# TritonDataCenter/containerpilot

Measured on AMD Instinct MI355X. Metric: events/sec, higher is better.
Workload: dtype n/a (CPU daemon, no tensor math; see BASELINE.json north_star); 1 GPU; model=containerpilot daemon, BASELINE stress shape scaled to 550 jobs, jobs=550, watches=50, parallelism=1 independent daemons (1/rank)

## Files before the change

### cpp/include/cpilot/loop.hpp

```cpp
#pragma once

#include <sys/types.h>

#include <chrono>
#include <cstdint>
#include <deque>
#include <functional>
#include <map>
#include <memory>
#include <mutex>
#include <queue>
#include <vector>

namespace cpilot {

using Clock = std::chrono::steady_clock;
using TimePoint = Clock::time_point;
using Ns = std::chrono::nanoseconds;

std::function<void()> timedItem(const char* tag, std::function<void()> fn);
void dumpItemTags();

void resetThreadScheduling();

class Loop {
 public:
  using FdCallback = std::function<void(uint32_t epollEvents)>;
  using TimerCallback = std::function<void()>;
  using ChildCallback = std::function<void(int waitStatus)>;

  Loop();
  ~Loop();

  Loop(const Loop&) = delete;
  Loop& operator=(const Loop&) = delete;

  void watchFd(int fd, uint32_t events, FdCallback cb);
  void modifyFd(int fd, uint32_t events);
  void unwatchFd(int fd);

  uint64_t addTimeout(Ns delay, TimerCallback cb);
  uint64_t addInterval(Ns interval, TimerCallback cb, Ns initialDelay = Ns(-1));
  void cancelTimer(uint64_t id);

  void defer(std::function<void()> fn);

  void post(std::function<void()> fn);

  void watchChild(pid_t pid, ChildCallback cb);
  void reapChildren();
  void notifyChildExit(pid_t pid, int status);

  static void postIfLive(Loop* loop, uint64_t id, std::function<void()> fn);
  uint64_t id() const { return id_; }

  void run();
  void stop();

  bool stopped() const { return stopped_; }

 private:
  struct Timer {
    uint64_t id;
    TimePoint deadline;
    Ns interval;
    TimerCallback cb;
    bool canceled = false;
  };
  struct TimerCmp {
    bool operator()(const std::shared_ptr<Timer>& a,
                    const std::shared_ptr<Timer>& b) const {
      return a->deadline > b->deadline;
    }
  };

  void armTimerFd();
  void fireDueTimers();
  void drainDeferred();
  void drainPosted();

  uint64_t id_ = 0;
  int epfd_ = -1;
  int timerfd_ = -1;
  int wakeupFds_[2] = {-1, -1};
  bool stopped_ = false;

  std::map<int, FdCallback> fdCallbacks_;
  std::priority_queue<std::shared_ptr<Timer>,
                      std::vector<std::shared_ptr<Timer>>, TimerCmp>
      timers_;
  std::map<uint64_t, std::shared_ptr<Timer>> timersById_;
  uint64_t nextTimerId_ = 1;

  std::deque<std::function<void()>> deferred_;

  std::mutex postedMu_;
  std::deque<std::function<void()>> posted_;

  std::map<pid_t, ChildCallback> children_;
  std::map<pid_t, int> unclaimedExits_;
};

}
```

### cpp/src/command.cpp

```cpp
#include "cpilot/command.hpp"

#include <fcntl.h>
#include <signal.h>
#include <sys/epoll.h>
#include <sys/wait.h>
#include <unistd.h>

#include <cctype>
#include <cstring>
#include <cstdio>
#include <map>

#include "cpilot/log.hpp"
#include "cpilot/spawner.hpp"

extern char** environ;

namespace cpilot {

namespace {

std::map<std::string, std::string>& pidEnvOverlay() {
  static std::map<std::string, std::string> overlay;
  return overlay;
}

std::shared_ptr<const std::vector<std::string>>& baseEnvCache() {
  static std::shared_ptr<const std::vector<std::string>> cache;
  return cache;
}
bool& baseEnvDirty() {
  static bool dirty = true;
  return dirty;
}

std::shared_ptr<const std::vector<std::string>> baseEnvSnapshot() {
  if (!baseEnvDirty() && baseEnvCache()) return baseEnvCache();
  auto& overlay = pidEnvOverlay();
  auto env = std::make_shared<std::vector<std::string>>();
  for (char** e = ::environ; *e; e++) {
    const char* eq = strchr(*e, '=');
    if (eq && overlay.count(std::string(*e, eq - *e))) continue;
    env->emplace_back(*e);
  }
  baseEnvCache() = env;
  baseEnvDirty() = false;
  return baseEnvCache();
}

std::vector<std::string>& overlayStrings() {
  static std::vector<std::string> strings;
  return strings;
}
std::map<std::string, size_t>& overlayIndex() {
  static std::map<std::string, size_t> index;
  return index;
}

const std::vector<std::string>& overlayExtras() { return overlayStrings(); }

void overlaySet(const std::string& key, const std::string& value) {
  auto [it, inserted] = pidEnvOverlay().emplace(key, value);
  if (inserted) {
    overlayIndex()[key] = overlayStrings().size();
    overlayStrings().push_back(key + "=" + value);
    if (getenv(key.c_str())) baseEnvDirty() = true;
  } else {
    it->second = value;
    overlayStrings()[overlayIndex()[key]] = key + "=" + value;
  }
}

void overlayErase(const std::string& key) {
  if (pidEnvOverlay().erase(key)) {
    auto idxIt = overlayIndex().find(key);
    if (idxIt != overlayIndex().end()) {
      size_t slot = idxIt->second;
      overlayIndex().erase(idxIt);
      auto& strs = overlayStrings();
      if (slot + 1 != strs.size()) {
        strs[slot] = std::move(strs.back());
        size_t eq = strs[slot].find('=');
        overlayIndex()[strs[slot].substr(0, eq)] = slot;
      }
      strs.pop_back();
    }
    if (getenv(key.c_str())) baseEnvDirty() = true;
  }
}

}

void commandEnvInvalidate() { baseEnvDirty() = true; }

bool parseArgs(const Json& raw, std::string* execPath,
               std::vector<std::string>* args, std::string* err) {
  std::vector<std::string> all;
  if (raw.isString()) {
    std::string s = raw.str();
    size_t a = 0, b = s.size();
    while (a < b && isspace((unsigned char)s[a])) a++;
    while (b > a && isspace((unsigned char)s[b - 1])) b--;
    s = s.substr(a, b - a);
    if (!s.empty()) {
      std::string cur;
      for (char c : s) {
        if (c == ' ') {
          all.push_back(cur);
          cur.clear();
        } else {
          cur += c;
        }
      }
      all.push_back(cur);
    }
  } else if (raw.isArray()) {
    for (auto& e : raw.array()) {
      if (e.isString()) all.push_back(e.str());
      else all.push_back(e.dump());
    }
  } else if (!raw.isNull()) {
    *err = "unable to parse exec arguments";
    return false;
  }
  if (all.empty()) {
    *err = "received zero-length argument";
    return false;
  }
  *execPath = all[0];
  args->assign(all.begin() + 1, all.end());
  return true;
}

CommandPtr newCommand(const Json& rawExec, Duration timeout, bool raw,
                      const std::string& logField, std::string* err) {
  std::string execPath;
  std::vector<std::string> args;
  if (!parseArgs(rawExec, &execPath, &args, err)) return nullptr;
  return std::make_shared<Command>(execPath, args, timeout, raw, logField);
}

Command::Command(std::string execPath, std::vector<std::string> args,
                 Duration timeout, bool raw, std::string logField)
    : name_(execPath),
      exec_(std::move(execPath)),
      args_(std::move(args)),
      timeout_(timeout),
      raw_(raw),
      logField_(std::move(logField)) {}

std::string Command::envName() const {
  if (name_.empty()) return name_;
  std::string name = name_;
  size_t slash = name.find_last_of('/');
  if (slash != std::string::npos) name = name.substr(slash + 1);
  size_t dot = name.find_last_of('.');
  if (dot != std::string::npos && dot > 0)
    name = name.substr(0, dot) + name.substr(name.size());
  std::string out;
  for (char c : name) {
    if (isalnum((unsigned char)c)) {
      out += (char)toupper((unsigned char)c);
    } else if (out.empty() || out.back() != '_') {
      out += '_';
    }
  }
  return out;
}

void Command::run(Loop& loop, std::shared_ptr<Bus> bus) {
  if (running_) {
    LOG_DEBUG("%s already running, queueing run", name_.c_str());
    pendingRun_ = true;
    return;
  }
  spawn(loop, std::move(bus));
}

void Command::spawn(Loop& loop, std::shared_ptr<Bus> bus) {
  loop_ = &loop;
  LOG_DEBUG("%s.Run start", name_.c_str());

  int pipefds[2] = {-1, -1};
  if (!raw_) {
    if (pipe2(pipefds, O_CLOEXEC) != 0) {
      LOG_ERROR("unable to create pipe for %s: %s", name_.c_str(),
                strerror(errno));
      bus->publish(Event{EventCode::ExitFailed, name_});
      bus->publish(Event{EventCode::Error, strerror(errno)});
      return;
    }
  }

  running_ = true;
  pid_ = -1;
  pendingSignal_ = 0;
  tReq_ = Clock::now();
  auto self = shared_from_this();
  int readFd = pipefds[0];
  auto baseEnv = baseEnvSnapshot();
  Spawner::SpawnCb compCb =
      [this, self, bus, readFd](pid_t pid, int err) {
        if (pid < 0) {
          LOG_ERROR("unable to start %s: %s", name_.c_str(), strerror(err));
          if (readFd >= 0) close(readFd);
          running_ = false;
          pendingRun_ = false;
          pendingSignal_ = 0;
          bus->publish(Event{EventCode::ExitFailed, name_});
          bus->publish(Event{EventCode::Error, strerror(err)});
          return;
        }
        pid_ = pid;
        tCb_ = Clock::now();
        if (pidEnvName_.empty())
          pidEnvName_ = "CONTAINERPILOT_" + envName() + "_PID";
        overlaySet(pidEnvName_, std::to_string(pid));

        if (!raw_) {
          logFd_ = readFd;
          fcntl(logFd_, F_SETFL, O_NONBLOCK);
          loop_->watchFd(logFd_, EPOLLIN | EPOLLHUP, [this, self](uint32_t) {
            char buf[4096];
            while (true) {
              ssize_t n = read(logFd_, buf, sizeof(buf));
              if (n > 0) {
                logBuf_.append(buf, n);
                size_t pos;
                while ((pos = logBuf_.find('\n')) != std::string::npos) {
                  logging::logFields(logging::Level::Info, logField_, pid_,
                                     logBuf_.substr(0, pos));
                  logBuf_.erase(0, pos + 1);
                }
              } else if (n == 0 || (n < 0 && errno != EAGAIN)) {
                if (!logBuf_.empty()) {
                  logging::logFields(logging::Level::Info, logField_, pid_,
                                     logBuf_);
                  logBuf_.clear();
                }
                loop_->unwatchFd(logFd_);
                close(logFd_);
                logFd_ = -1;
                return;
              } else {
                return;
              }
            }
          });
        }

        if (timeout_ > Duration(0)) {
          timeoutTimer_ = loop_->addTimeout(timeout_, [this, self] {
            LOG_WARN("%s timeout after %llds", name_.c_str(),
                     (long long)std::chrono::duration_cast<
                         std::chrono::seconds>(timeout_)
                         .count());
            timeoutTimer_ = 0;
            kill();
          });
        }

        if (pendingSignal_ != 0) {
          ::kill(-pid, pendingSignal_);
          pendingSignal_ = 0;
        }

        loop_->watchChild(pid, [this, self, bus](int status) {
          onExit(*loop_, bus, status);
        });
      };
  Spawner::global().spawn(loop, exec_, args_, std::move(baseEnv),
                          overlayExtras(), raw_ ? -1 : pipefds[1],
                          std::move(compCb));
}

void Command::onExit(Loop& loop, std::shared_ptr<Bus> bus, int status) {
  LOG_DEBUG("%s.Run end", name_.c_str());
  static const bool rttDebug = cpilotDebugEnv("CPILOT_LOOP_DEBUG");
  if (rttDebug) {
    auto now = Clock::now();
    double total =
        std::chrono::duration<double, std::milli>(now - tReq_).count();
    if (total > 50.0) {
      double execPhase =
          std::chrono::duration<double, std::milli>(now - tCb_).count();
      fprintf(stderr,
              "spawn rtt: %s total=%.0fms spawn_phase=%.0fms "
              "exec_phase=%.0fms\n",
              name_.c_str(), total, total - execPhase, execPhase);
    }
  }
  if (timeoutTimer_) {
    loop.cancelTimer(timeoutTimer_);
    timeoutTimer_ = 0;
  }
  if (logFd_ >= 0) {
    char buf[4096];
    ssize_t n;
    while ((n = read(logFd_, buf, sizeof(buf))) > 0) logBuf_.append(buf, n);
    size_t pos;
    while ((pos = logBuf_.find('\n')) != std::string::npos) {
      logging::logFields(logging::Level::Info, logField_, pid_,
                         logBuf_.substr(0, pos));
      logBuf_.erase(0, pos + 1);
    }
    if (!logBuf_.empty()) {
      logging::logFields(logging::Level::Info, logField_, pid_, logBuf_);
      logBuf_.clear();
    }
    loop.unwatchFd(logFd_);
    close(logFd_);
    logFd_ = -1;
  }

  if (!pidEnvName_.empty()) overlayErase(pidEnvName_);

  running_ = false;
  pid_ = -1;

  bool success = WIFEXITED(status) && WEXITSTATUS(status) == 0;
  if (success) {
    LOG_DEBUG("%s exited without error", name_.c_str());
    bus->publish(Event{EventCode::ExitSuccess, name_});
  } else {
    int code = WIFEXITED(status) ? WEXITSTATUS(status)
                                 : 128 + (WIFSIGNALED(status) ? WTERMSIG(status) : 0);
    LOG_ERROR("%s exited with error: exit status %d", name_.c_str(), code);
    bus->publish(Event{EventCode::ExitFailed, name_});
    bus->publish(Event{EventCode::Error,
                      name_ + ": exit status " + std::to_string(code)});
  }

  if (pendingRun_) {
    pendingRun_ = false;
    spawn(loop, bus);
  }
}

void Command::term() {
  LOG_DEBUG("%s.term", name_.c_str());
  if (pid_ > 0) {
    LOG_DEBUG("terminating command '%s' at pid: %d", name_.c_str(), pid_);
    ::kill(-pid_, SIGTERM);
  } else if (running_ && pendingSignal_ != SIGKILL) {
    pendingSignal_ = SIGTERM;
  }
}

void Command::kill() {
  LOG_DEBUG("%s.kill", name_.c_str());
  if (pid_ > 0) {
    LOG_DEBUG("killing command '%s' at pid: %d", name_.c_str(), pid_);
    ::kill(-pid_, SIGKILL);
  } else if (running_) {
    pendingSignal_ = SIGKILL;
  }
}

}
```

### cpp/src/loop.cpp

```cpp
#include "cpilot/loop.hpp"

#include <fcntl.h>
#include <sched.h>
#include <sys/resource.h>
#include <sys/epoll.h>
#include <sys/timerfd.h>
#include <sys/wait.h>
#include <unistd.h>

#include <cstdio>
#include <cstring>
#include <algorithm>
#include <set>
#include <stdexcept>

#include "cpilot/log.hpp"

namespace cpilot {

void resetThreadScheduling() {
  struct sched_param sp;
  memset(&sp, 0, sizeof(sp));
  sched_setscheduler(0, SCHED_OTHER, &sp);
  setpriority(PRIO_PROCESS, 0, 0);
}

namespace {
std::mutex& liveLoopsMu() {
  static std::mutex mu;
  return mu;
}
std::map<Loop*, uint64_t>& liveLoops() {
  static std::map<Loop*, uint64_t> loops;
  return loops;
}
uint64_t nextLoopId() {
  static uint64_t next = 1;
  return next++;
}
}

namespace {
struct ItemTagStats {
  double ms = 0;
  uint64_t count = 0;
};
std::map<std::string, ItemTagStats>& itemTags() {
  static std::map<std::string, ItemTagStats> tags;
  return tags;
}
}

std::function<void()> timedItem(const char* tag, std::function<void()> fn) {
  static const bool on = cpilotDebugEnv("CPILOT_LOOP_DEBUG");
  if (!on) return fn;
  std::string t(tag);
  return [t, fn = std::move(fn)] {
    TimePoint t0 = Clock::now();
    fn();
    auto& slot = itemTags()[t];
    slot.ms +=
        std::chrono::duration<double, std::milli>(Clock::now() - t0).count();
    slot.count++;
  };
}

void dumpItemTags() {
  for (auto& kv : itemTags())
    fprintf(stderr, "  item tag %s: %.0fms over %llu (avg %.1fus)\n",
            kv.first.c_str(), kv.second.ms,
            (unsigned long long)kv.second.count,
            kv.second.count ? kv.second.ms * 1000 / kv.second.count : 0.0);
  itemTags().clear();
}

void Loop::postIfLive(Loop* loop, uint64_t id, std::function<void()> fn) {
  std::lock_guard<std::mutex> l(liveLoopsMu());
  auto it = liveLoops().find(loop);
  if (it != liveLoops().end() && it->second == id) loop->post(std::move(fn));
}

Loop::Loop() {
  {
    std::lock_guard<std::mutex> l(liveLoopsMu());
    id_ = nextLoopId();
    liveLoops()[this] = id_;
  }
  epfd_ = epoll_create1(EPOLL_CLOEXEC);
  if (epfd_ < 0) throw std::runtime_error("epoll_create1 failed");
  timerfd_ = timerfd_create(CLOCK_MONOTONIC, TFD_NONBLOCK | TFD_CLOEXEC);
  if (timerfd_ < 0) throw std::runtime_error("timerfd_create failed");
  if (pipe2(wakeupFds_, O_NONBLOCK | O_CLOEXEC) != 0)
    throw std::runtime_error("pipe2 failed");

  watchFd(timerfd_, EPOLLIN, [this](uint32_t) {
    uint64_t expirations;
    while (read(timerfd_, &expirations, sizeof(expirations)) > 0) {
    }
    fireDueTimers();
  });
  watchFd(wakeupFds_[0], EPOLLIN, [this](uint32_t) {
    char buf[256];
    while (read(wakeupFds_[0], buf, sizeof(buf)) > 0) {
    }
    drainPosted();
  });
}

Loop::~Loop() {
  {
    std::lock_guard<std::mutex> l(liveLoopsMu());
    liveLoops().erase(this);
  }
  if (epfd_ >= 0) close(epfd_);
  if (timerfd_ >= 0) close(timerfd_);
  if (wakeupFds_[0] >= 0) close(wakeupFds_[0]);
  if (wakeupFds_[1] >= 0) close(wakeupFds_[1]);
}

void Loop::watchFd(int fd, uint32_t events, FdCallback cb) {
  struct epoll_event ev;
  memset(&ev, 0, sizeof(ev));
  ev.events = events;
  ev.data.fd = fd;
  if (epoll_ctl(epfd_, EPOLL_CTL_ADD, fd, &ev) != 0)
    throw std::runtime_error(std::string("epoll_ctl ADD failed: ") +
                             strerror(errno));
  fdCallbacks_[fd] = std::move(cb);
}

void Loop::modifyFd(int fd, uint32_t events) {
  struct epoll_event ev;
  memset(&ev, 0, sizeof(ev));
  ev.events = events;
  ev.data.fd = fd;
  epoll_ctl(epfd_, EPOLL_CTL_MOD, fd, &ev);
}

void Loop::unwatchFd(int fd) {
  epoll_ctl(epfd_, EPOLL_CTL_DEL, fd, nullptr);
  fdCallbacks_.erase(fd);
}

uint64_t Loop::addTimeout(Ns delay, TimerCallback cb) {
  auto t = std::make_shared<Timer>();
  t->id = nextTimerId_++;
  t->deadline = Clock::now() + delay;
  t->interval = Ns(0);
  t->cb = std::move(cb);
  timersById_[t->id] = t;
  timers_.push(t);
  armTimerFd();
  return t->id;
}

uint64_t Loop::addInterval(Ns interval, TimerCallback cb, Ns initialDelay) {
  if (interval <= Ns(0)) interval = Ns(1);
  if (initialDelay < Ns(0)) initialDelay = interval;
  auto t = std::make_shared<Timer>();
  t->id = nextTimerId_++;
  t->deadline = Clock::now() + initialDelay;
  t->interval = interval;
  t->cb = std::move(cb);
  timersById_[t->id] = t;
  timers_.push(t);
  armTimerFd();
  return t->id;
}

void Loop::cancelTimer(uint64_t id) {
  auto it = timersById_.find(id);
  if (it == timersById_.end()) return;
  it->second->canceled = true;
  timersById_.erase(it);
}

void Loop::defer(std::function<void()> fn) { deferred_.push_back(std::move(fn)); }

void Loop::post(std::function<void()> fn) {
  {
    std::lock_guard<std::mutex> l(postedMu_);
    posted_.push_back(std::move(fn));
  }
  char b = 1;
  ssize_t unused = write(wakeupFds_[1], &b, 1);
  (void)unused;
}

void Loop::watchChild(pid_t pid, ChildCallback cb) {
  auto it = unclaimedExits_.find(pid);
  if (it != unclaimedExits_.end()) {
    int status = it->second;
    unclaimedExits_.erase(it);
    cb(status);
    return;
  }
  children_[pid] = std::move(cb);
}

void Loop::reapChildren() {
  constexpr int kReapBatch = 64;
  int n = 0;
  while (n < kReapBatch) {
    int status = 0;
    pid_t pid = waitpid(-1, &status, WNOHANG);
    if (pid <= 0) return;
    n++;
    notifyChildExit(pid, status);
  }
  defer([this] { reapChildren(); });
}

void Loop::notifyChildExit(pid_t pid, int status) {
  auto it = children_.find(pid);
  if (it != children_.end()) {
    ChildCallback cb = std::move(it->second);
    children_.erase(it);
    cb(status);
  } else {
    unclaimedExits_[pid] = status;
  }
}

void Loop::armTimerFd() {
  while (!timers_.empty() && timers_.top()->canceled) timers_.pop();
  struct itimerspec its;
  memset(&its, 0, sizeof(its));
  if (!timers_.empty()) {
    auto now = Clock::now();
    Ns delta = std::chrono::duration_cast<Ns>(timers_.top()->deadline - now);
    if (delta < Ns(1)) delta = Ns(1);
    its.it_value.tv_sec = delta.count() / 1000000000LL;
    its.it_value.tv_nsec = delta.count() % 1000000000LL;
  }
  timerfd_settime(timerfd_, 0, &its, nullptr);
}

void Loop::fireDueTimers() {
  static const bool stallDebug = cpilotDebugEnv("CPILOT_LOOP_DEBUG");
  auto timeCb = [](Timer* t, const TimerCallback& cb) {
    if (!stallDebug) { cb(); return; }
    TimePoint t0 = Clock::now();
    cb();
    auto ms = std::chrono::duration<double, std::milli>(Clock::now() - t0)
                  .count();
    if (ms > 10.0)
      fprintf(stderr, "timer stall: id=%llu interval_ms=%lld took %.1f ms\n",
              (unsigned long long)t->id,
              (long long)(t->interval.count() / 1000000), ms);
  };
  auto now = Clock::now();
  while (!timers_.empty()) {
    auto t = timers_.top();
    if (t->canceled) {
      timers_.pop();
      continue;
    }
    if (t->deadline > now) break;
    timers_.pop();
    if (t->interval > Ns(0)) {
      t->deadline += t->interval;
      if (t->deadline <= now) {
        auto behind = std::chrono::duration_cast<Ns>(now - t->deadline);
        auto periods = behind.count() / t->interval.count() + 1;
        t->deadline += Ns(periods * t->interval.count());
      }
      timers_.push(t);
      timeCb(t.get(), t->cb);
    } else {
      auto keep = t;
      timersById_.erase(t->id);
      timeCb(keep.get(), keep->cb);
    }
  }
  armTimerFd();
}

void Loop::drainDeferred() {
  size_t n = deferred_.size();
  for (size_t i = 0; i < n && !deferred_.empty(); i++) {
    auto fn = std::move(deferred_.front());
    deferred_.pop_front();
    fn();
  }
}

void Loop::drainPosted() {
  constexpr auto kBudget = std::chrono::milliseconds(2);
  constexpr size_t kHardCap = 4096;
  TimePoint start = Clock::now();
  size_t processed = 0;
  bool more = true;
  while (more && processed < kHardCap &&
         Clock::now() - start < kBudget) {
    std::deque<std::function<void()>> batch;
    {
      std::lock_guard<std::mutex> l(postedMu_);
      for (size_t i = 0; i < 64 && !posted_.empty(); i++) {
        batch.push_back(std::move(posted_.front()));
        posted_.pop_front();
      }
      more = !posted_.empty();
    }
    static const bool itemDebug = cpilotDebugEnv("CPILOT_LOOP_DEBUG");
    if (itemDebug) {
      static double accMs = 0;
      static uint64_t nItems = 0, nSlow = 0;
      static TimePoint lastDump = Clock::now();
      for (auto& fn : batch) {
        TimePoint ti = Clock::now();
        fn();
        double ms = std::chrono::duration<double, std::milli>(
                        Clock::now() - ti).count();
        accMs += ms;
        nItems++;
        if (ms > 0.2) nSlow++;
      }
      if (Clock::now() - lastDump > std::chrono::seconds(5)) {
        fprintf(stderr,
                "posted items: %llu in 5s, total=%.0fms avg=%.1fus "
                "slow(>200us)=%llu\n",
                (unsigned long long)nItems, accMs,
                nItems ? accMs * 1000.0 / nItems : 0.0,
                (unsigned long long)nSlow);
        accMs = 0;
        nItems = nSlow = 0;
        lastDump = Clock::now();
      }
    } else {
      for (auto& fn : batch) fn();
    }
    processed += batch.size();
    if (batch.empty()) break;
  }
  if (more) {
    char b = 1;
    ssize_t unused = write(wakeupFds_[1], &b, 1);
    (void)unused;
  }
}

void Loop::run() {
  stopped_ = false;
  const bool stallDebug = cpilotDebugEnv("CPILOT_LOOP_DEBUG");
  auto probe = [stallDebug](const char* phase, TimePoint t0, int fd = -1) {
    if (!stallDebug) return;
    auto ms = std::chrono::duration<double, std::milli>(Clock::now() - t0)
                  .count();
    if (ms > 10.0)
      fprintf(stderr, "loop stall: %s fd=%d took %.1f ms\n", phase, fd, ms);
  };
  std::vector<struct epoll_event> events(64);
  double accDeferred = 0, accEpoll = 0, accFds = 0, accTimers = 0;
  std::map<int, std::pair<double, uint64_t>> accPerFd;
  uint64_t iters = 0;
  TimePoint lastReport = Clock::now();
  auto acc = [](double* slot, TimePoint t0) {
    *slot += std::chrono::duration<double, std::milli>(Clock::now() - t0)
                 .count();
  };
  while (!stopped_) {
    TimePoint t0 = Clock::now();
    drainDeferred();
    probe("drainDeferred", t0);
    if (stallDebug) acc(&accDeferred, t0);
    if (stopped_) break;
    armTimerFd();
    int timeoutMs = deferred_.empty() ? 1000 : 0;
    TimePoint te = Clock::now();
    int n = epoll_wait(epfd_, events.data(), (int)events.size(), timeoutMs);
    if (stallDebug) acc(&accEpoll, te);
    if (n < 0) {
      if (errno == EINTR) continue;
      LOG_ERROR("epoll_wait: %s", strerror(errno));
      break;
    }
    TimePoint tf = Clock::now();
    for (int i = 0; i < n && !stopped_; i++) {
      int fd = events[i].data.fd;
      auto it = fdCallbacks_.find(fd);
      if (it != fdCallbacks_.end()) {
        FdCallback cb = it->second;
        TimePoint tc = Clock::now();
        cb(events[i].events);
        probe("fdCallback", tc, fd);
        if (stallDebug) {
          auto& slot = accPerFd[fd];
          slot.first += std::chrono::duration<double, std::milli>(
                            Clock::now() - tc).count();
          slot.second++;
        }
      }
    }
    if (stallDebug) acc(&accFds, tf);
    TimePoint tt = Clock::now();
    fireDueTimers();
    probe("fireDueTimers", tt);
    if (stallDebug) {
      acc(&accTimers, tt);
      iters++;
      if (Clock::now() - lastReport > std::chrono::seconds(5)) {
        double secs = std::chrono::duration<double>(Clock::now() -
                                                    lastReport).count();
        fprintf(stderr,
                "loop phases: %.0f it/s deferred=%.0fms epoll=%.0fms "
                "fds=%.0fms timers=%.0fms (per %.1fs)\n",
                iters / secs, accDeferred, accEpoll, accFds, accTimers,
                secs);
        std::vector<std::pair<double, std::pair<int, uint64_t>>> top;
        for (auto& kv : accPerFd)
          top.push_back({kv.second.first, {kv.first, kv.second.second}});
        std::sort(top.rbegin(), top.rend());
        for (size_t k = 0; k < top.size() && k < 4; k++)
          fprintf(stderr, "  top fd %d: %.0fms over %llu events\n",
                  top[k].second.first, top[k].first,
                  (unsigned long long)top[k].second.second);
        dumpItemTags();
        accPerFd.clear();
        accDeferred = accEpoll = accFds = accTimers = 0;
        iters = 0;
        lastReport = Clock::now();
      }
    }
  }
}

void Loop::stop() { stopped_ = true; }

}
```

Before: 11000 events/s.

## Skip redundant timerfd rearming and cheapen PID env overlay updates

```diff
diff --git a/cpp/include/cpilot/loop.hpp b/cpp/include/cpilot/loop.hpp
--- a/cpp/include/cpilot/loop.hpp
+++ b/cpp/include/cpilot/loop.hpp
@@ -59,6 +59,8 @@
 
   bool stopped() const { return stopped_; }
 
+  uint64_t timerArmCount() const { return timerArmCount_; }
+
  private:
   struct Timer {
     uint64_t id;
@@ -91,6 +93,8 @@
       timers_;
   std::map<uint64_t, std::shared_ptr<Timer>> timersById_;
   uint64_t nextTimerId_ = 1;
+  int64_t armedDeadlineNs_ = 0;
+  uint64_t timerArmCount_ = 0;
 
   std::deque<std::function<void()>> deferred_;
 
diff --git a/cpp/src/command.cpp b/cpp/src/command.cpp
--- a/cpp/src/command.cpp
+++ b/cpp/src/command.cpp
@@ -9,7 +9,7 @@
 #include <cctype>
 #include <cstring>
 #include <cstdio>
-#include <map>
+#include <unordered_map>
 
 #include "cpilot/log.hpp"
 #include "cpilot/spawner.hpp"
@@ -20,9 +20,31 @@
 
 namespace {
 
-std::map<std::string, std::string>& pidEnvOverlay() {
-  static std::map<std::string, std::string> overlay;
-  return overlay;
+struct OverlaySlot {
+  static constexpr size_t kAbsent = (size_t)-1;
+  size_t index = kAbsent;
+  std::string parked;
+  int inEnviron = -1;
+};
+std::unordered_map<std::string, OverlaySlot>& overlaySlots() {
+  static std::unordered_map<std::string, OverlaySlot> slots;
+  return slots;
+}
+std::vector<std::string>& overlayStrings() {
+  static std::vector<std::string> strings;
+  return strings;
+}
+std::vector<OverlaySlot*>& overlayOwners() {
+  static std::vector<OverlaySlot*> owners;
+  return owners;
+}
+
+const std::vector<std::string>& overlayExtras() { return overlayStrings(); }
+
+bool overlayHas(const std::string& key) {
+  auto it = overlaySlots().find(key);
+  return it != overlaySlots().end() &&
+         it->second.index != OverlaySlot::kAbsent;
 }
 
 std::shared_ptr<const std::vector<std::string>>& baseEnvCache() {
@@ -36,11 +58,10 @@
 
 std::shared_ptr<const std::vector<std::string>> baseEnvSnapshot() {
   if (!baseEnvDirty() && baseEnvCache()) return baseEnvCache();
-  auto& overlay = pidEnvOverlay();
   auto env = std::make_shared<std::vector<std::string>>();
   for (char** e = ::environ; *e; e++) {
     const char* eq = strchr(*e, '=');
-    if (eq && overlay.count(std::string(*e, eq - *e))) continue;
+    if (eq && overlayHas(std::string(*e, eq - *e))) continue;
     env->emplace_back(*e);
   }
   baseEnvCache() = env;
@@ -48,51 +69,65 @@
   return baseEnvCache();
 }
 
-std::vector<std::string>& overlayStrings() {
-  static std::vector<std::string> strings;
-  return strings;
-}
-std::map<std::string, size_t>& overlayIndex() {
-  static std::map<std::string, size_t> index;
-  return index;
-}
-
-const std::vector<std::string>& overlayExtras() { return overlayStrings(); }
-
-void overlaySet(const std::string& key, const std::string& value) {
-  auto [it, inserted] = pidEnvOverlay().emplace(key, value);
-  if (inserted) {
-    overlayIndex()[key] = overlayStrings().size();
-    overlayStrings().push_back(key + "=" + value);
-    if (getenv(key.c_str())) baseEnvDirty() = true;
+bool shadowsEnviron(const std::string& key, OverlaySlot& slot) {
+  if (slot.inEnviron < 0) slot.inEnviron = getenv(key.c_str()) ? 1 : 0;
+  return slot.inEnviron == 1;
+}
+
+void overlaySet(const std::string& key, pid_t pid) {
+  char value[16];
+  int n = snprintf(value, sizeof(value), "%d", (int)pid);
+  OverlaySlot& slot = overlaySlots()[key];
+  if (slot.index == OverlaySlot::kAbsent) {
+    std::string kv = std::move(slot.parked);
+    kv.assign(key);
+    kv.push_back('=');
+    kv.append(value, n);
+    slot.index = overlayStrings().size();
+    overlayStrings().push_back(std::move(kv));
+    overlayOwners().push_back(&slot);
+    if (shadowsEnviron(key, slot)) baseEnvDirty() = true;
   } else {
-    it->second = value;
-    overlayStrings()[overlayIndex()[key]] = key + "=" + value;
+    std::string& kv = overlayStrings()[slot.index];
+    kv.resize(key.size() + 1);
+    kv.append(value, n);
   }
 }
 
 void overlayErase(const std::string& key) {
-  if (pidEnvOverlay().erase(key)) {
-    auto idxIt = overlayIndex().find(key);
-    if (idxIt != overlayIndex().end()) {
-      size_t slot = idxIt->second;
-      overlayIndex().erase(idxIt);
-      auto& strs = overlayStrings();
-      if (slot + 1 != strs.size()) {
-        strs[slot] = std::move(strs.back());
-        size_t eq = strs[slot].find('=');
-        overlayIndex()[strs[slot].substr(0, eq)] = slot;
-      }
-      strs.pop_back();
-    }
-    if (getenv(key.c_str())) baseEnvDirty() = true;
-  }
-}
-
-}
-
-void commandEnvInvalidate() { baseEnvDirty() = true; }
-
+  auto it = overlaySlots().find(key);
+  if (it == overlaySlots().end()) return;
+  OverlaySlot& slot = it->second;
+  if (slot.index == OverlaySlot::kAbsent) return;
+  auto& strs = overlayStrings();
+  auto& owners = overlayOwners();
+  size_t i = slot.index;
+  slot.parked = std::move(strs[i]);
+  if (i + 1 != strs.size()) {
+    strs[i] = std::move(strs.back());
+    owners[i] = owners.back();
+    owners[i]->index = i;
+  }
+  strs.pop_back();
+  owners.pop_back();
+  slot.index = OverlaySlot::kAbsent;
+  if (shadowsEnviron(key, slot)) baseEnvDirty() = true;
+}
+
+}
+
+void commandEnvInvalidate() {
+  baseEnvDirty() = true;
+  auto& slots = overlaySlots();
+  for (auto it = slots.begin(); it != slots.end();) {
+    if (it->second.index == OverlaySlot::kAbsent) {
+      it = slots.erase(it);
+    } else {
+      it->second.inEnviron = -1;
+      ++it;
+    }
+  }
+}
 bool parseArgs(const Json& raw, std::string* execPath,
                std::vector<std::string>* args, std::string* err) {
   std::vector<std::string> all;
@@ -215,7 +250,7 @@
         tCb_ = Clock::now();
         if (pidEnvName_.empty())
           pidEnvName_ = "CONTAINERPILOT_" + envName() + "_PID";
-        overlaySet(pidEnvName_, std::to_string(pid));
+        overlaySet(pidEnvName_, pid);
 
         if (!raw_) {
           logFd_ = readFd;
diff --git a/cpp/src/loop.cpp b/cpp/src/loop.cpp
--- a/cpp/src/loop.cpp
+++ b/cpp/src/loop.cpp
@@ -96,6 +96,7 @@
   watchFd(timerfd_, EPOLLIN, [this](uint32_t) {
     uint64_t expirations;
     while (read(timerfd_, &expirations, sizeof(expirations)) > 0) {
+      armedDeadlineNs_ = 0;
     }
     fireDueTimers();
   });
@@ -224,16 +225,20 @@
 
 void Loop::armTimerFd() {
   while (!timers_.empty() && timers_.top()->canceled) timers_.pop();
+  int64_t want = 0;
+  if (!timers_.empty()) {
+    want = std::chrono::duration_cast<Ns>(
+               timers_.top()->deadline.time_since_epoch()).count();
+    if (want < 1) want = 1;
+  }
+  if (want == armedDeadlineNs_) return;
   struct itimerspec its;
   memset(&its, 0, sizeof(its));
-  if (!timers_.empty()) {
-    auto now = Clock::now();
-    Ns delta = std::chrono::duration_cast<Ns>(timers_.top()->deadline - now);
-    if (delta < Ns(1)) delta = Ns(1);
-    its.it_value.tv_sec = delta.count() / 1000000000LL;
-    its.it_value.tv_nsec = delta.count() % 1000000000LL;
-  }
-  timerfd_settime(timerfd_, 0, &its, nullptr);
+  its.it_value.tv_sec = want / 1000000000LL;
+  its.it_value.tv_nsec = want % 1000000000LL;
+  timerfd_settime(timerfd_, TFD_TIMER_ABSTIME, &its, nullptr);
+  armedDeadlineNs_ = want;
+  timerArmCount_++;
 }
 
 void Loop::fireDueTimers() {
@@ -354,6 +359,7 @@
   double accDeferred = 0, accEpoll = 0, accFds = 0, accTimers = 0;
   std::map<int, std::pair<double, uint64_t>> accPerFd;
   uint64_t iters = 0;
+  uint64_t lastArmCount = timerArmCount_;
   TimePoint lastReport = Clock::now();
   auto acc = [](double* slot, TimePoint t0) {
     *slot += std::chrono::duration<double, std::milli>(Clock::now() - t0)
@@ -404,9 +410,11 @@
                                                     lastReport).count();
         fprintf(stderr,
                 "loop phases: %.0f it/s deferred=%.0fms epoll=%.0fms "
-                "fds=%.0fms timers=%.0fms (per %.1fs)\n",
+                "fds=%.0fms timers=%.0fms timerfd_settime=%llu "
+                "(per %.1fs)\n",
                 iters / secs, accDeferred, accEpoll, accFds, accTimers,
-                secs);
+                (unsigned long long)(timerArmCount_ - lastArmCount), secs);
+        lastArmCount = timerArmCount_;
         std::vector<std::pair<double, std::pair<int, uint64_t>>> top;
         for (auto& kv : accPerFd)
           top.push_back({kv.second.first, {kv.first, kv.second.second}});
```

Measured after the change: 11000 events/s. About the same (-0.0%).
